# Shigangli/Ok-Topk

Hardware: NVIDIA H100
Metric: train_samples_per_sec_vgg16_oktopk_density0.001 (higher is better)
Workload: dtype fp32

## Files before the change

### oktopk_b200/csrc/bindings.cpp

```cpp
#include <pybind11/pybind11.h>
#include <pybind11/stl.h>
#include <cuda.h>
#include <cuda_runtime.h>

#include <unistd.h>

#include <algorithm>
#include <cstring>
#include <stdexcept>
#include <string>
#include <tuple>
#include <vector>

#include "oktopk.cuh"

namespace py = pybind11;
using namespace okt;

static void ck(cudaError_t e, const char* what) {
    if (e != cudaSuccess) throw std::runtime_error(std::string(what) + ": " + cudaGetErrorString(e));
}
template <class T> static T* P_(uint64_t p) { return reinterpret_cast<T*>(p); }
static cudaStream_t S_(uint64_t s) { return reinterpret_cast<cudaStream_t>(s); }

// ... 438 lines not shown
static void fused_adam(uint64_t p, uint64_t g, uint64_t m, uint64_t v, int n, double beta1, double beta2, double eps,
                       double wd, int decoupled, int zero_grad, uint64_t stream, uint64_t scal_ptr, uint64_t fault_ptr,
                       uint64_t skip_ptr) {
    if (scal_ptr == 0) throw std::runtime_error("fused_adam: scal_ptr must point at the group's device scalars");
    ck(launch_fused_adam(P_<float>(p), P_<float>(g), P_<float>(m), P_<float>(v), n, beta1, beta2, (float)eps, (float)wd,
                         decoupled, zero_grad, P_<float>(scal_ptr), P_<int>(fault_ptr), P_<int>(skip_ptr), S_(stream)),
       "fused_adam");
}
static BnDtype bn_dtype(int dtype, const char* what) {
    if (dtype < 0 || dtype > 2) throw std::runtime_error(std::string(what) + ": dtype must be 0 (fp32), 1 (bf16) or 2 (fp16)");
    return static_cast<BnDtype>(dtype);
}
static void bn_forward(uint64_t x, uint64_t y, uint64_t arg, uint64_t partial, uint64_t gamma, uint64_t beta, uint64_t cbias,
                       uint64_t save_mean, uint64_t save_invstd, uint64_t rmean, uint64_t rvar, uint64_t nbt, double momentum,
                       double eps, int relu, int M, int C, int W, int slot, int max_ctas, uint64_t stream, int dtype,
                       uint64_t res) {
    if (C % 4 != 0) throw std::runtime_error("bn_forward: channel count must be a multiple of 4");
    if (slot < 0) throw std::runtime_error("bn_forward: negative slot");
    if (res != 0 && (W != 0 || !relu)) throw std::runtime_error("bn_forward: a residual needs relu = 1 and no pool");
    ck(launch_bn_forward(P_<const void>(x), P_<void>(y), P_<unsigned char>(arg), P_<float>(partial), P_<const float>(gamma),
                         P_<const float>(beta), P_<const float>(cbias), P_<float>(save_mean), P_<float>(save_invstd),
                         P_<float>(rmean), P_<float>(rvar), P_<long long>(nbt), (float)momentum, (float)eps, relu, M, C, W, slot,
                         max_ctas, bn_dtype(dtype, "bn_forward"), S_(stream), P_<const void>(res)), "bn_forward");
}
static void bn_backward(uint64_t x, uint64_t dy, uint64_t arg, uint64_t dx, uint64_t partial, uint64_t gamma, uint64_t beta,
                        uint64_t save_mean, uint64_t save_invstd, uint64_t dgamma, uint64_t dbeta, int relu, int M, int C, int W,
                        int slot, int max_ctas, uint64_t stream, int dtype, uint64_t res, uint64_t dres) {
    if (slot < 0) throw std::runtime_error("bn_backward: negative slot");
    if ((res == 0) != (dres == 0)) throw std::runtime_error("bn_backward: res and dres go together");
    if (res != 0 && (W != 0 || !relu)) throw std::runtime_error("bn_backward: a residual needs relu = 1 and no pool");
    ck(launch_bn_backward(P_<const void>(x), P_<const void>(dy), P_<const unsigned char>(arg), P_<void>(dx), P_<float>(partial),
                          P_<const float>(gamma), P_<const float>(beta), P_<const float>(save_mean), P_<const float>(save_invstd),
                          P_<float>(dgamma), P_<float>(dbeta), relu, M, C, W, slot, max_ctas, bn_dtype(dtype, "bn_backward"),
                          S_(stream), P_<const void>(res), P_<void>(dres)), "bn_backward");
}
static void maxpool2_fwd(uint64_t x, uint64_t y, uint64_t arg, int N, int H, int W, int C, uint64_t stream) {
    if ((C % 4) || (H % 2) || (W % 2)) throw std::runtime_error("maxpool2_fwd: needs C % 4 == 0 and even H, W");
    ck(launch_maxpool2_fwd(P_<const float>(x), P_<float>(y), P_<unsigned char>(arg), N, H, W, C, S_(stream)), "maxpool2_fwd");
}
static void maxpool2_bwd(uint64_t dy, uint64_t arg, uint64_t dx, int N, int H, int W, int C, uint64_t stream) {
    ck(launch_maxpool2_bwd(P_<const float>(dy), P_<const unsigned char>(arg), P_<float>(dx), N, H, W, C, S_(stream)), "maxpool2_bwd");
}
static void momentum_correct(uint64_t g, uint64_t buf, int n, double momentum, uint64_t stream) {
    ck(launch_momentum_correct(P_<float>(g), P_<float>(buf), n, (float)momentum, S_(stream)), "momentum_correct");
}
static void clip_by_norm(uint64_t x, int n, uint64_t scratch, double max_norm, uint64_t stream) {
    ck(launch_l2norm_sq(P_<float>(x), n, P_<float>(scratch), S_(stream)), "l2norm");
    ck(launch_scale(P_<float>(x), n, P_<float>(scratch), (float)max_norm, S_(stream)), "clip scale");
}
// ... 89 lines not shown
    m.def("adam_scalars", [](uint64_t ls, uint64_t hyper, uint64_t scal, int groups, uint64_t stream) {
        ck(launch_adam_scalars(P_<const LossScaleDev>(ls), P_<const double>(hyper), P_<float>(scal), groups, S_(stream)),
           "adam_scalars");
    });
    m.def("carry_residual", [](uint64_t g, uint64_t res, int n, uint64_t skip, uint64_t stream) {
        ck(launch_carry_residual(P_<float>(g), P_<float>(res), n, P_<const int>(skip), S_(stream)), "carry_residual");
    });
    m.attr("LOSS_SCALE_BYTES") = sizeof(LossScaleDev);
    m.attr("SCALE_SYNC_BYTES") = sizeof(ScaleSync);
    m.attr("VERDICT_OFFSET") = offsetof(ScaleSync, verdict);
    m.def("maxpool2_fwd", &maxpool2_fwd);
    m.def("maxpool2_bwd", &maxpool2_bwd);
    m.def("bn_forward", &bn_forward, py::arg("x"), py::arg("y"), py::arg("arg"), py::arg("partial"), py::arg("gamma"),
          py::arg("beta"), py::arg("cbias"), py::arg("save_mean"), py::arg("save_invstd"), py::arg("rmean"), py::arg("rvar"),
          py::arg("nbt"), py::arg("momentum"), py::arg("eps"), py::arg("relu"), py::arg("M"), py::arg("C"), py::arg("W"),
          py::arg("slot"), py::arg("max_ctas"), py::arg("stream"), py::arg("dtype"), py::arg("res") = 0);
    m.def("bn_backward", &bn_backward, py::arg("x"), py::arg("dy"), py::arg("arg"), py::arg("dx"), py::arg("partial"),
          py::arg("gamma"), py::arg("beta"), py::arg("save_mean"), py::arg("save_invstd"), py::arg("dgamma"), py::arg("dbeta"),
          py::arg("relu"), py::arg("M"), py::arg("C"), py::arg("W"), py::arg("slot"), py::arg("max_ctas"), py::arg("stream"),
          py::arg("dtype"), py::arg("res") = 0, py::arg("dres") = 0);
    m.def("bn_tile_rows", &bn_tile_rows);
    m.def("clip_by_norm", &clip_by_norm);
    m.attr("MAXP") = OKT_MAXP;
    m.attr("TRACE_LEN") = kTraceLen;
    m.attr("LAND_MAX") = kLandMax;
    m.attr("SRC_SEG_MAX") = kSrcSegMax;
    m.attr("CHUNK") = kChunk;
}
```

### oktopk_b200/csrc/bnrelu.cu

```cuda
#include <cuda_bf16.h>
#include <cuda_fp16.h>

#include "common.cuh"
#include "oktopk.cuh"

namespace okt {

constexpr int kBnThreads = 256;
constexpr int kBnMaxBlocks = 512;
constexpr int kBnHold = 8;
constexpr int kBnSyncSlots = 1024;

__device__ unsigned int g_bn_sync[kBnSyncSlots][2];

struct BnGeom {
    int M, C, cv;
    int tpr, rpi;
    int rows_per_block, nblk;
    int hold;
    int W;
};

__host__ __device__ inline BnGeom bn_geom(int M, int C) {
    BnGeom g;
    g.M = M; g.C = C; g.cv = C >> 2;
    g.tpr = g.cv < kBnThreads ? g.cv : kBnThreads;
// ... 90 lines not shown
    if (ty < g.rpi) { s_red[ty * g.tpr + tx] = s; s_red[(g.rpi + ty) * g.tpr + tx] = q; }
    __syncthreads();
    if (ty == 0 && col < g.cv) {
        for (int j = 1; j < g.rpi; ++j) {
            const float4 a = s_red[j * g.tpr + tx], b = s_red[(g.rpi + j) * g.tpr + tx];
            s.x += a.x; s.y += a.y; s.z += a.z; s.w += a.w;
            q.x += b.x; q.y += b.y; q.z += b.z; q.w += b.w;
        }
        float4* p4 = reinterpret_cast<float4*>(partial + (size_t)tile * 2 * g.C);
        p4[col] = s;
        p4[g.cv + col] = q;
    }
    __syncthreads();
}

__device__ __forceinline__ bool bn_arrive(unsigned int* sync, unsigned int& gen) {
    __shared__ unsigned int s_gen;
    __shared__ int s_last;
    __syncthreads();
    if (threadIdx.x == 0) {
        s_gen = ld_acquire_gpu_u32(sync + 1);
        const unsigned int old = atom_add_acq_rel_gpu_u32(sync, 1u);
        s_last = old == gridDim.x - 1u;
        if (s_last) st_relaxed_gpu_u32(sync, 0u);
    }
    __syncthreads();
    gen = s_gen;
    return s_last != 0;
}

__device__ __forceinline__ void bn_release(unsigned int* sync, bool last, unsigned int gen) {
    __syncthreads();
    if (threadIdx.x == 0) {
        if (last) {
            st_release_gpu_u32(sync + 1, gen + 1u);
        } else {
            while (ld_acquire_gpu_u32(sync + 1) == gen) { }
        }
    }
    __syncthreads();
}

template <typename T>
struct BnFwdArgs {
    const T* x;
    T* y;
    unsigned char* arg;
    float* partial;
    const float* gamma; const float* beta; const float* cbias;
    float* save_mean; float* save_invstd; float* rmean; float* rvar; long long* nbt;
    float momentum, eps;
    int relu;
    unsigned int* sync;
    BnGeom g;
    const T* res;
};

template <bool kPool, bool kRes, typename T>
__global__ void __launch_bounds__(kBnThreads) bn_fwd_kernel(const BnFwdArgs<T> p) {
    static_assert(!(kPool && kRes), "no pool follows a residual add");
    using A = BnAct<T>;
    using V = typename A::V;
    extern __shared__ float4 s_dyn[];
    __shared__ float4 s_red[2 * kBnThreads];
    const BnGeom& g = p.g;
    const int tx = threadIdx.x % g.tpr, ty = threadIdx.x / g.tpr;
    const V* x4 = reinterpret_cast<const V*>(p.x);
    auto ldx = [&](size_t o) { return A::wide(__ldg(x4 + o)); };
    const size_t st1 = (size_t)g.rpi * g.cv;
    V h[kBnHold];

    for (int t = blockIdx.x; t < g.nblk; t += gridDim.x) {
        const bool held = g.hold && t == (int)blockIdx.x;
        const int row0 = t * g.rows_per_block, row1 = min(g.M, row0 + g.rows_per_block);
        for (int c0 = 0; c0 < g.cv; c0 += g.tpr) {
            const int col = c0 + tx;
            float4 s = make_float4(0.f, 0.f, 0.f, 0.f), q = s;
            if (ty < g.rpi && col < g.cv) {
                auto acc = [&](const float4& v) {
                    s.x += v.x; s.y += v.y; s.z += v.z; s.w += v.w;
// ... 9 lines not shown
                        if (r + k * g.rpi < row1) acc(A::wide(h[k]));
                } else {
                    for (; r + 3 * g.rpi < row1; r += 4 * g.rpi) {
                        const size_t o = (size_t)r * g.cv + col;
                        const float4 v0 = ldx(o), v1 = ldx(o + st1), v2 = ldx(o + 2 * st1), v3 = ldx(o + 3 * st1);
                        acc(v0); acc(v1); acc(v2); acc(v3);
                    }
                    for (; r < row1; r += g.rpi) acc(ldx((size_t)r * g.cv + col));
                }
            }
            bn_tile_partial(s, q, tx, ty, col, g, s_red, p.partial, t);
        }
    }

    float* s_ab = reinterpret_cast<float*>(s_dyn);
    unsigned int gen;
    const bool last = bn_arrive(p.sync, gen);
    if (last) {
        float* s_tot = s_ab;
        bn_combine_partials(p.partial, g.nblk, g.C, s_tot, s_red);
        for (int c = threadIdx.x; c < g.C; c += kBnThreads) {
            const double s = (double)s_tot[c], q = (double)s_tot[g.C + c];
            const double mean = s / (double)g.M;
            double var = q / (double)g.M - mean * mean;
            if (var < 0.0) var = 0.0;
            const float invstd = (float)(1.0 / sqrt(var + (double)p.eps));
            p.save_mean[c] = (float)mean;
            p.save_invstd[c] = invstd;
            if (p.rmean != nullptr) {
                const float mb = (float)mean + (p.cbias != nullptr ? __ldg(p.cbias + c) : 0.f);
                const double unb = g.M > 1 ? var * (double)g.M / (double)(g.M - 1) : var;
                p.rmean[c] = fmaf(p.momentum, mb, __fmul_rn(1.f - p.momentum, p.rmean[c]));
                p.rvar[c] = fmaf(p.momentum, (float)unb, __fmul_rn(1.f - p.momentum, p.rvar[c]));
            }
        }
        if (threadIdx.x == 0 && p.nbt != nullptr) *p.nbt += 1;
    }
    bn_release(p.sync, last, gen);
    for (int c = threadIdx.x; c < g.C; c += kBnThreads) {
        const float a = __fmul_rn(__ldg(p.gamma + c), __ldcg(p.save_invstd + c));
        s_ab[c] = a;
        s_ab[g.C + c] = __fsub_rn(__ldg(p.beta + c), __fmul_rn(__ldcg(p.save_mean + c), a));
    }
    __syncthreads();

    const float4* ab4 = s_dyn;
    auto yval = [&](const float4& xin, int col) {
        float4 v = f4_fma(xin, ab4[col], ab4[g.cv + col]);
        if (p.relu) { v.x = fmaxf(v.x, 0.f); v.y = fmaxf(v.y, 0.f); v.z = fmaxf(v.z, 0.f); v.w = fmaxf(v.w, 0.f); }
        return v;
    };
    const V* r4 = reinterpret_cast<const V*>(p.res);
    auto ldr = [&](size_t o) { return A::wide(__ldg(r4 + o)); };
    auto yres = [&](const float4& xin, const float4& rin, int col) {
        float4 v = f4_fma(xin, ab4[col], ab4[g.cv + col]);
        v.x += rin.x; v.y += rin.y; v.z += rin.z; v.w += rin.w;
        v.x = fmaxf(v.x, 0.f); v.y = fmaxf(v.y, 0.f); v.z = fmaxf(v.z, 0.f); v.w = fmaxf(v.w, 0.f);
// ... 77 lines not shown
struct BnBwdArgs {
    const T* x;
    const T* dy;
    const unsigned char* arg;
    T* dx;
    float* partial;
    const float* gamma; const float* beta; const float* save_mean; const float* save_invstd;
    float* dgamma; float* dbeta;
    int relu;
    unsigned int* sync;
    BnGeom g;
    const T* res;
    T* dres;
};

template <bool kPool, bool kRes, typename T>
__global__ void __launch_bounds__(kBnThreads) bn_bwd_kernel(const BnBwdArgs<T> p) {
    static_assert(!(kPool && kRes), "no pool follows a residual add");
    using A = BnAct<T>;
    using V = typename A::V;
    extern __shared__ float4 s_dyn[];
    __shared__ float4 s_red[2 * kBnThreads];
    const BnGeom& g = p.g;
    const int tx = threadIdx.x % g.tpr, ty = threadIdx.x / g.tpr;
    const V* x4 = reinterpret_cast<const V*>(p.x);
    const V* d4 = reinterpret_cast<const V*>(p.dy);
    const uchar4* a4 = reinterpret_cast<const uchar4*>(p.arg);
    auto ldx = [&](size_t o) { return A::wide(__ldg(x4 + o)); };
    const size_t st1 = (size_t)g.rpi * g.cv;
    auto grad = [&](int row0, int r, int col) -> float4 {
        if (!kPool) return A::wide(__ldg(d4 + (size_t)r * g.cv + col));
        const int lr = r - row0, hl = lr / g.W, w = lr - hl * g.W;
        const size_t o = (size_t)(row0 / 4 + (hl >> 1) * (g.W >> 1) + (w >> 1)) * g.cv + col;
        const int k = (hl & 1) * 2 + (w & 1);
        const float4 d = A::wide(__ldg(d4 + o));
        const uchar4 a = __ldg(a4 + o);
        return make_float4(a.x == k ? d.x : 0.f, a.y == k ? d.y : 0.f, a.z == k ? d.z : 0.f, a.w == k ? d.w : 0.f);
    };
// ... 85 lines not shown
                            const size_t o = (size_t)r * g.cv + col;
                            const float4 v = ldx(o);
                            float4 e = grad(row0, r, col);
                            gate(k, v, ldr(o), o, e);
                            acc(v, e);
                        } else {
                            acc(ldx((size_t)r * g.cv + col), grad(row0, r, col));
                        }
                    }
                }
            }
            bn_tile_partial(sb, sg, tx, ty, col, g, s_red, p.partial, t);
        }
    }

    unsigned int gen;
    const bool last = bn_arrive(p.sync, gen);
    if (last) {
        float* s_tot = reinterpret_cast<float*>(s_dyn);
        bn_combine_partials(p.partial, g.nblk, g.C, s_tot, s_red);
        for (int c = threadIdx.x; c < g.C; c += kBnThreads) { p.dbeta[c] = s_tot[c]; p.dgamma[c] = s_tot[g.C + c]; }
    }
    bn_release(p.sync, last, gen);

    for (int t = blockIdx.x; t < g.nblk; t += gridDim.x) {
        const bool held = g.hold && t == (int)blockIdx.x;
        const int row0 = t * g.rows_per_block, row1 = min(g.M, row0 + g.rows_per_block);
        for (int c0 = 0; c0 < g.cv; c0 += g.tpr) {
            const int col = c0 + tx;
            if (ty >= g.rpi || col >= g.cv) continue;
            const Col k = column(col);
            const float4 db = __ldcg(reinterpret_cast<const float4*>(p.dbeta) + col);
            const float4 dg = __ldcg(reinterpret_cast<const float4*>(p.dgamma) + col);
            const double M = (double)g.M;
            const float4 mb = make_float4((float)(db.x / M), (float)(db.y / M), (float)(db.z / M), (float)(db.w / M));
            const float4 mg = make_float4((float)(dg.x / M), (float)(dg.y / M), (float)(dg.z / M), (float)(dg.w / M));
            V* o4 = reinterpret_cast<V*>(p.dx);
            auto out = [&](size_t off, const float4& v, float4 d) {
                const float4 xh = xhat(k, v);
                if constexpr (!kRes) mask(k, v, d);
                o4[off] = A::narrow(make_float4(k.a.x * (d.x - mb.x - xh.x * mg.x), k.a.y * (d.y - mb.y - xh.y * mg.y),
                                                k.a.z * (d.z - mb.z - xh.z * mg.z), k.a.w * (d.w - mb.w - xh.w * mg.w)));
            };
            int r = row0 + ty;
            if (held) {
#pragma unroll
                for (int j = 0; j < kBnHold; ++j)
                    if (r + j * g.rpi < row1) out((size_t)(r + j * g.rpi) * g.cv + col, A::wide(hx[j]), hd[j]);
// ... 18 lines not shown

static unsigned int* bn_sync_slot(int slot) {
    static unsigned int* base[64] = {nullptr};
    int dev = 0;
    cudaGetDevice(&dev);
    if (dev < 0 || dev >= 64) return nullptr;
    if (base[dev] == nullptr) {
        void* a = nullptr;
        if (cudaGetSymbolAddress(&a, g_bn_sync) != cudaSuccess) return nullptr;
        base[dev] = static_cast<unsigned int*>(a);
    }
    return base[dev] + 2 * (size_t)(slot % kBnSyncSlots);
}

template <typename Args>
static cudaError_t bn_launch(void (*kernel)(const Args), Args p, size_t smem, int max_ctas, cudaStream_t stream) {
    int dev = 0, sms = 0, per = 0;
    cudaGetDevice(&dev);
    cudaError_t e = cudaDeviceGetAttribute(&sms, cudaDevAttrMultiProcessorCount, dev);
    if (e == cudaSuccess && smem > 32 * 1024)
        e = cudaFuncSetAttribute(kernel, cudaFuncAttributeMaxDynamicSharedMemorySize, (int)smem);
    if (e == cudaSuccess) e = cudaOccupancyMaxActiveBlocksPerMultiprocessor(&per, kernel, kBnThreads, smem);
    if (e != cudaSuccess) return e;
    if (per < 1) return cudaErrorInvalidConfiguration;
    int grid = p.g.nblk < per * sms ? p.g.nblk : per * sms;
    if (max_ctas > 0 && grid > max_ctas) grid = max_ctas;
    void* args[] = {(void*)&p};
    e = cudaLaunchCooperativeKernel((void*)kernel, dim3(grid), dim3(kBnThreads), args, smem, stream);
    (void)cudaGetLastError();
    return e;
}

static cudaError_t bn_prepare(BnGeom& g, unsigned int*& sync, int M, int C, int W, int slot) {
    g = bn_geom(M, C);
    g.W = W;
    if (W > 0 && (W % 2 != 0 || g.rows_per_block % (2 * W) != 0 || M % (2 * W) != 0)) return cudaErrorInvalidValue;
    sync = bn_sync_slot(slot);
    return sync == nullptr ? cudaErrorInvalidDevice : cudaSuccess;
}

template <typename T>
static cudaError_t bn_forward_t(const void* x, void* y, unsigned char* arg, float* partial, const float* gamma,
                                const float* beta, const float* cbias, float* save_mean, float* save_invstd, float* rmean,
                                float* rvar, long long* nbt, float momentum, float eps, int relu, int M, int C, int W, int slot,
                                int max_ctas, cudaStream_t stream, const void* res) {
    if (res != nullptr && (W > 0 || !relu)) return cudaErrorInvalidValue;
    BnFwdArgs<T> p{static_cast<const T*>(x), static_cast<T*>(y), arg, partial, gamma, beta, cbias, save_mean, save_invstd,
                   rmean, rvar, nbt, momentum, eps, relu, nullptr, {}, static_cast<const T*>(res)};
    cudaError_t e = bn_prepare(p.g, p.sync, M, C, W, slot);
    if (e != cudaSuccess) return e;
    size_t smem = sizeof(float) * 2 * C;
    if (W > 0 && p.g.hold) smem += sizeof(float4) * p.g.rows_per_block * p.g.cv;
    if (W > 0) return bn_launch(bn_fwd_kernel<true, false, T>, p, smem, max_ctas, stream);
    return res != nullptr ? bn_launch(bn_fwd_kernel<false, true, T>, p, smem, max_ctas, stream)
                          : bn_launch(bn_fwd_kernel<false, false, T>, p, smem, max_ctas, stream);
}

template <typename T>
static cudaError_t bn_backward_t(const void* x, const void* dy, const unsigned char* arg, void* dx, float* partial,
                                 const float* gamma, const float* beta, const float* save_mean, const float* save_invstd,
                                 float* dgamma, float* dbeta, int relu, int M, int C, int W, int slot, int max_ctas,
                                 cudaStream_t stream, const void* res, void* dres) {
    if ((res == nullptr) != (dres == nullptr) || (res != nullptr && (W > 0 || !relu))) return cudaErrorInvalidValue;
    BnBwdArgs<T> p{static_cast<const T*>(x), static_cast<const T*>(dy), arg, static_cast<T*>(dx), partial, gamma, beta,
                   save_mean, save_invstd, dgamma, dbeta, relu, nullptr, {}, static_cast<const T*>(res),
                   static_cast<T*>(dres)};
    cudaError_t e = bn_prepare(p.g, p.sync, M, C, W, slot);
    if (e != cudaSuccess) return e;
    const size_t smem = sizeof(float) * 2 * C;
    if (W > 0) return bn_launch(bn_bwd_kernel<true, false, T>, p, smem, max_ctas, stream);
    return res != nullptr ? bn_launch(bn_bwd_kernel<false, true, T>, p, smem, max_ctas, stream)
                          : bn_launch(bn_bwd_kernel<false, false, T>, p, smem, max_ctas, stream);
}

cudaError_t launch_bn_forward(const void* x, void* y, unsigned char* arg, float* partial, const float* gamma, const float* beta,
                              const float* cbias, float* save_mean, float* save_invstd, float* rmean, float* rvar, long long* nbt,
                              float momentum, float eps, int relu, int M, int C, int W, int slot, int max_ctas, BnDtype dtype,
                              cudaStream_t stream, const void* res) {
    switch (dtype) {
        case BnDtype::kF32:
            return bn_forward_t<float>(x, y, arg, partial, gamma, beta, cbias, save_mean, save_invstd, rmean, rvar, nbt,
                                       momentum, eps, relu, M, C, W, slot, max_ctas, stream, res);
        case BnDtype::kBF16:
            return bn_forward_t<__nv_bfloat16>(x, y, arg, partial, gamma, beta, cbias, save_mean, save_invstd, rmean, rvar,
                                               nbt, momentum, eps, relu, M, C, W, slot, max_ctas, stream, res);
        case BnDtype::kF16:
            return bn_forward_t<__half>(x, y, arg, partial, gamma, beta, cbias, save_mean, save_invstd, rmean, rvar, nbt,
                                        momentum, eps, relu, M, C, W, slot, max_ctas, stream, res);
    }
    return cudaErrorInvalidValue;
}

cudaError_t launch_bn_backward(const void* x, const void* dy, const unsigned char* arg, void* dx, float* partial,
                               const float* gamma, const float* beta, const float* save_mean, const float* save_invstd,
                               float* dgamma, float* dbeta, int relu, int M, int C, int W, int slot, int max_ctas, BnDtype dtype,
                               cudaStream_t stream, const void* res, void* dres) {
    switch (dtype) {
        case BnDtype::kF32:
            return bn_backward_t<float>(x, dy, arg, dx, partial, gamma, beta, save_mean, save_invstd, dgamma, dbeta, relu,
                                        M, C, W, slot, max_ctas, stream, res, dres);
        case BnDtype::kBF16:
            return bn_backward_t<__nv_bfloat16>(x, dy, arg, dx, partial, gamma, beta, save_mean, save_invstd, dgamma, dbeta,
                                                relu, M, C, W, slot, max_ctas, stream, res, dres);
        case BnDtype::kF16:
            return bn_backward_t<__half>(x, dy, arg, dx, partial, gamma, beta, save_mean, save_invstd, dgamma, dbeta, relu,
                                         M, C, W, slot, max_ctas, stream, res, dres);
    }
    return cudaErrorInvalidValue;
}

}

namespace okt {

constexpr int kPoolThreads = 256;

__global__ void __launch_bounds__(kPoolThreads) maxpool2_fwd_kernel(const float* __restrict__ x, float* __restrict__ y,
                                                                     unsigned char* __restrict__ arg, int N, int H, int W,
                                                                     int C) {
    const int cv = C >> 2, Ho = H >> 1, Wo = W >> 1;
    const long long total = (long long)N * Ho * Wo * cv;
// ... 70 lines not shown
```

### oktopk_b200/csrc/common.cuh

```cuda
#pragma once
#include <cuda_runtime.h>
#include <stdint.h>

#ifndef OKT_MAXP
#define OKT_MAXP 16
#endif

namespace okt {

__device__ __forceinline__ unsigned long long globaltimer_ns() {
    unsigned long long t;
    asm volatile("mov.u64 %0, %%globaltimer;" : "=l"(t));
    return t;
}

__device__ __forceinline__ void st_release_sys_u64(uint64_t* p, uint64_t v) {
    asm volatile("st.release.sys.global.u64 [%0], %1;" ::"l"(p), "l"(v) : "memory");
}
__device__ __forceinline__ uint64_t ld_acquire_sys_u64(const uint64_t* p) {
    uint64_t v;
    asm volatile("ld.acquire.sys.global.u64 %0, [%1];" : "=l"(v) : "l"(p) : "memory");
    return v;
}
__device__ __forceinline__ uint64_t ld_relaxed_sys_u64(const uint64_t* p) {
// ... 8 lines not shown
    asm volatile("st.relaxed.sys.global.u64 [%0], %1;" ::"l"(p), "l"(v) : "memory");
}
__device__ __forceinline__ uint32_t ld_relaxed_sys_u32(const uint32_t* p) {
    uint32_t v;
    asm volatile("ld.relaxed.sys.global.u32 %0, [%1];" : "=r"(v) : "l"(p) : "memory");
    return v;
}
__device__ __forceinline__ unsigned long long ld_acquire_gpu_u64(const unsigned long long* p) {
    unsigned long long v;
    asm volatile("ld.acquire.gpu.global.u64 %0, [%1];" : "=l"(v) : "l"(p) : "memory");
    return v;
}
__device__ __forceinline__ uint32_t ld_acquire_gpu_u32(const uint32_t* p) {
    uint32_t v;
    asm volatile("ld.acquire.gpu.global.u32 %0, [%1];" : "=r"(v) : "l"(p) : "memory");
    return v;
}
__device__ __forceinline__ void st_release_gpu_u32(uint32_t* p, uint32_t v) {
    asm volatile("st.release.gpu.global.u32 [%0], %1;" ::"l"(p), "r"(v) : "memory");
}
__device__ __forceinline__ void st_relaxed_gpu_u32(uint32_t* p, uint32_t v) {
    asm volatile("st.relaxed.gpu.global.u32 [%0], %1;" ::"l"(p), "r"(v) : "memory");
}
__device__ __forceinline__ uint32_t atom_add_acq_rel_gpu_u32(uint32_t* p, uint32_t v) {
    uint32_t old;
    asm volatile("atom.acq_rel.gpu.global.add.u32 %0, [%1], %2;" : "=r"(old) : "l"(p), "r"(v) : "memory");
    return old;
}
__device__ __forceinline__ void fence_acq_rel_sys() { asm volatile("fence.acq_rel.sys;" ::: "memory"); }
__device__ __forceinline__ void fence_acq_rel_gpu() { asm volatile("fence.acq_rel.gpu;" ::: "memory"); }
// ... 189 lines not shown
```

### oktopk_b200/csrc/oktopk.cuh

```cuda
#pragma once
#include <cuda_runtime.h>
#include <stdint.h>
#include <stddef.h>

#ifndef OKT_MAXP
#define OKT_MAXP 16
#endif

namespace okt {

constexpr int kThreads = 512;
constexpr int kWarps = kThreads / 32;
constexpr int kChunk = 1024;
constexpr int kHistBins = 2048;
constexpr int kMaxWarpsTotal = 16384;
constexpr int kGuardMax = 64;
constexpr int kGuardFineMax = 15;
constexpr int kCtasPerSm = 1;
constexpr int kPackTile = 2;
constexpr int kPackStages = 4;
constexpr int kPackSmemBytes = kPackStages * 2 * kPackTile * kThreads * 16;
constexpr int kScanStages = 2 * kPackStages;
constexpr int kStrideGridMax = 132 * 8;

// ... 262 lines not shown
cudaError_t launch_carry_residual(float* g, float* res, int n, const int* skip, cudaStream_t stream);
constexpr int kLandMax = 96;
struct LandParams {
    const float* src[kLandMax];
    long long dst_off[kLandMax];
    int numel[kLandMax];
    int blk_begin[kLandMax + 1];
    int count;
};
cudaError_t launch_land(const LandParams& lp, float* bucket, cudaStream_t stream);
enum class BnDtype : int { kF32 = 0, kBF16 = 1, kF16 = 2 };
int bn_tile_rows(int M, int C);
cudaError_t launch_bn_forward(const void* x, void* y, unsigned char* arg, float* partial, const float* gamma, const float* beta,
                              const float* cbias, float* save_mean, float* save_invstd, float* rmean, float* rvar, long long* nbt,
                              float momentum, float eps, int relu, int M, int C, int W, int slot, int max_ctas, BnDtype dtype,
                              cudaStream_t stream, const void* res = nullptr);
cudaError_t launch_bn_backward(const void* x, const void* dy, const unsigned char* arg, void* dx, float* partial,
                               const float* gamma, const float* beta, const float* save_mean, const float* save_invstd,
                               float* dgamma, float* dbeta, int relu, int M, int C, int W, int slot, int max_ctas, BnDtype dtype,
                               cudaStream_t stream, const void* res = nullptr, void* dres = nullptr);
cudaError_t launch_maxpool2_fwd(const float* x, float* y, unsigned char* arg, int N, int H, int W, int C, cudaStream_t stream);
cudaError_t launch_maxpool2_bwd(const float* dy, const unsigned char* arg, float* dx, int N, int H, int W, int C,
                                cudaStream_t stream);
cudaError_t launch_momentum_correct(float* g, float* buf, int n, float momentum, cudaStream_t stream);
cudaError_t launch_l2norm_sq(const float* x, int n, float* out, cudaStream_t stream);
cudaError_t launch_scale(float* x, int n, const float* norm_sq, float max_norm, cudaStream_t stream);

}
```

### oktopk_b200/ops/fused_bn.py

```python
from __future__ import annotations

import itertools
from typing import Optional

import torch
import torch.nn.functional as F

from . import ext

MAX_CTAS = 0

_SLOTS = itertools.count()

_DTYPE_FLAG = {torch.float32: 0, torch.bfloat16: 1, torch.float16: 2}


def _sync_slot(bn: torch.nn.BatchNorm2d) -> int:
    s = bn.__dict__.get("_okt_bn_slot")
    if s is None:
        s = bn.__dict__["_okt_bn_slot"] = next(_SLOTS)
    return s


def _dtype_ok(x: torch.Tensor, fp16: bool = False) -> bool:
    if not torch.is_autocast_enabled():
# ... 40 lines not shown
        dtype = _DTYPE_FLAG[x.dtype]
        if pool:
            y = torch.empty((N, Ch, H // 2, W // 2), dtype=x.dtype, device=x.device, memory_format=torch.channels_last)
            arg = torch.empty(y.numel(), dtype=torch.uint8, device=x.device)
        else:
            y = torch.empty_like(x)
            arg = None
        rows = C.bn_tile_rows(M, Ch)
        partial = torch.empty((M + rows - 1) // rows * 2 * Ch, dtype=torch.float32, device=x.device)
        stats = torch.empty(2 * Ch, dtype=torch.float32, device=x.device)
        s = torch.cuda.current_stream().cuda_stream
        C.bn_forward(x.data_ptr(), y.data_ptr(), 0 if arg is None else arg.data_ptr(), partial.data_ptr(), gamma.data_ptr(),
                     beta.data_ptr(), 0 if cbias is None else cbias.data_ptr(), stats.data_ptr(), stats.data_ptr() + 4 * Ch,
                     0 if rmean is None else rmean.data_ptr(), 0 if rvar is None else rvar.data_ptr(),
                     0 if nbt is None else nbt.data_ptr(), float(momentum), float(eps), int(relu), M, Ch,
                     W if pool else 0, slot, MAX_CTAS, s, dtype, 0 if res is None else res.data_ptr())
        ctx.save_for_backward(x, gamma, beta, stats, arg, res)
        ctx.relu, ctx.pool, ctx.slot, ctx.dtype = bool(relu), bool(pool), slot, dtype
        return y

    @staticmethod
    def backward(ctx, dy):
        C = ext.require()
        x, gamma, beta, stats, arg, res = ctx.saved_tensors
        N, Ch, H, W = x.shape
        M = N * H * W
        assert dy.dtype == x.dtype, (dy.dtype, x.dtype)
        if not dy.is_contiguous(memory_format=torch.channels_last):
            dy = dy.contiguous(memory_format=torch.channels_last)
        dx = torch.empty_like(x)
        rows = C.bn_tile_rows(M, Ch)
        partial = torch.empty((M + rows - 1) // rows * 2 * Ch, dtype=torch.float32, device=x.device)
        dgb = torch.empty(2 * Ch, dtype=torch.float32, device=x.device)
        dres = None if res is None else torch.empty_like(x)
        s = torch.cuda.current_stream().cuda_stream
        C.bn_backward(x.data_ptr(), dy.data_ptr(), 0 if arg is None else arg.data_ptr(), dx.data_ptr(), partial.data_ptr(),
                      gamma.data_ptr(), beta.data_ptr(), stats.data_ptr(), stats.data_ptr() + 4 * Ch, dgb.data_ptr(),
                      dgb.data_ptr() + 4 * Ch, int(ctx.relu), M, Ch, W if ctx.pool else 0, ctx.slot, MAX_CTAS, s,
                      ctx.dtype, 0 if res is None else res.data_ptr(), 0 if dres is None else dres.data_ptr())
        return dx, dgb[:Ch], dgb[Ch:], None, None, None, None, None, None, None, None, None, dres


def _check_residual(residual: Optional[torch.Tensor], relu: bool, pool: Optional[torch.nn.MaxPool2d]) -> None:
    if residual is not None and (not relu or pool is not None):
        raise ValueError("a residual is added before the ReLU: it needs relu=True and pool=None")


def bias_bn_relu(x: torch.Tensor, bn: torch.nn.BatchNorm2d, conv_bias: Optional[torch.Tensor] = None,
                 relu: bool = True, pool: Optional[torch.nn.MaxPool2d] = None, fp16: bool = False,
                 residual: Optional[torch.Tensor] = None) -> torch.Tensor:
    _check_residual(residual, relu, pool)
    if (_fast_path_ok(x, bn, fp16) and (conv_bias is None or conv_bias.dtype == torch.float32)
            and (residual is None or _residual_ok(x, residual))):
        if residual is not None and not residual.is_contiguous(memory_format=torch.channels_last):
# ... 96 lines not shown
```

Before: 13160.

## Let every CTA combine BN partials redundantly instead of last-block broadcast

Adds a variant of the fused BN forward and backward kernels in which every CTA waits at a grid barrier and then reduces all per-tile partials itself. The last CTA alone writes saved stats, running stats and dgamma/dbeta, while every CTA uses its own shared-memory copy. The old scheme had a serial combine by one CTA and a second global read of the stats after release. The variant is chosen when the tile count is at most 128, and it trades redundant reduction reads of the partials for a shorter critical path.

```diff
diff --git a/oktopk_b200/csrc/bindings.cpp b/oktopk_b200/csrc/bindings.cpp
--- a/oktopk_b200/csrc/bindings.cpp
+++ b/oktopk_b200/csrc/bindings.cpp
@@ -476,25 +476,25 @@
 static void bn_forward(uint64_t x, uint64_t y, uint64_t arg, uint64_t partial, uint64_t gamma, uint64_t beta, uint64_t cbias,
                        uint64_t save_mean, uint64_t save_invstd, uint64_t rmean, uint64_t rvar, uint64_t nbt, double momentum,
                        double eps, int relu, int M, int C, int W, int slot, int max_ctas, uint64_t stream, int dtype,
-                       uint64_t res) {
+                       uint64_t res, int all_tiles) {
     if (C % 4 != 0) throw std::runtime_error("bn_forward: channel count must be a multiple of 4");
     if (slot < 0) throw std::runtime_error("bn_forward: negative slot");
     if (res != 0 && (W != 0 || !relu)) throw std::runtime_error("bn_forward: a residual needs relu = 1 and no pool");
     ck(launch_bn_forward(P_<const void>(x), P_<void>(y), P_<unsigned char>(arg), P_<float>(partial), P_<const float>(gamma),
                          P_<const float>(beta), P_<const float>(cbias), P_<float>(save_mean), P_<float>(save_invstd),
                          P_<float>(rmean), P_<float>(rvar), P_<long long>(nbt), (float)momentum, (float)eps, relu, M, C, W, slot,
-                         max_ctas, bn_dtype(dtype, "bn_forward"), S_(stream), P_<const void>(res)), "bn_forward");
+                         max_ctas, bn_dtype(dtype, "bn_forward"), S_(stream), P_<const void>(res), all_tiles), "bn_forward");
 }
 static void bn_backward(uint64_t x, uint64_t dy, uint64_t arg, uint64_t dx, uint64_t partial, uint64_t gamma, uint64_t beta,
                         uint64_t save_mean, uint64_t save_invstd, uint64_t dgamma, uint64_t dbeta, int relu, int M, int C, int W,
-                        int slot, int max_ctas, uint64_t stream, int dtype, uint64_t res, uint64_t dres) {
+                        int slot, int max_ctas, uint64_t stream, int dtype, uint64_t res, uint64_t dres, int all_tiles) {
     if (slot < 0) throw std::runtime_error("bn_backward: negative slot");
     if ((res == 0) != (dres == 0)) throw std::runtime_error("bn_backward: res and dres go together");
     if (res != 0 && (W != 0 || !relu)) throw std::runtime_error("bn_backward: a residual needs relu = 1 and no pool");
     ck(launch_bn_backward(P_<const void>(x), P_<const void>(dy), P_<const unsigned char>(arg), P_<void>(dx), P_<float>(partial),
                           P_<const float>(gamma), P_<const float>(beta), P_<const float>(save_mean), P_<const float>(save_invstd),
                           P_<float>(dgamma), P_<float>(dbeta), relu, M, C, W, slot, max_ctas, bn_dtype(dtype, "bn_backward"),
-                          S_(stream), P_<const void>(res), P_<void>(dres)), "bn_backward");
+                          S_(stream), P_<const void>(res), P_<void>(dres), all_tiles), "bn_backward");
 }
 static void maxpool2_fwd(uint64_t x, uint64_t y, uint64_t arg, int N, int H, int W, int C, uint64_t stream) {
     if ((C % 4) || (H % 2) || (W % 2)) throw std::runtime_error("maxpool2_fwd: needs C % 4 == 0 and even H, W");
@@ -614,11 +614,12 @@
     m.def("bn_forward", &bn_forward, py::arg("x"), py::arg("y"), py::arg("arg"), py::arg("partial"), py::arg("gamma"),
           py::arg("beta"), py::arg("cbias"), py::arg("save_mean"), py::arg("save_invstd"), py::arg("rmean"), py::arg("rvar"),
           py::arg("nbt"), py::arg("momentum"), py::arg("eps"), py::arg("relu"), py::arg("M"), py::arg("C"), py::arg("W"),
-          py::arg("slot"), py::arg("max_ctas"), py::arg("stream"), py::arg("dtype"), py::arg("res") = 0);
+          py::arg("slot"), py::arg("max_ctas"), py::arg("stream"), py::arg("dtype"), py::arg("res") = 0,
+          py::arg("all_tiles") = -1);
     m.def("bn_backward", &bn_backward, py::arg("x"), py::arg("dy"), py::arg("arg"), py::arg("dx"), py::arg("partial"),
           py::arg("gamma"), py::arg("beta"), py::arg("save_mean"), py::arg("save_invstd"), py::arg("dgamma"), py::arg("dbeta"),
           py::arg("relu"), py::arg("M"), py::arg("C"), py::arg("W"), py::arg("slot"), py::arg("max_ctas"), py::arg("stream"),
-          py::arg("dtype"), py::arg("res") = 0, py::arg("dres") = 0);
+          py::arg("dtype"), py::arg("res") = 0, py::arg("dres") = 0, py::arg("all_tiles") = -1);
     m.def("bn_tile_rows", &bn_tile_rows);
     m.def("clip_by_norm", &clip_by_norm);
     m.attr("MAXP") = OKT_MAXP;
diff --git a/oktopk_b200/csrc/bnrelu.cu b/oktopk_b200/csrc/bnrelu.cu
--- a/oktopk_b200/csrc/bnrelu.cu
+++ b/oktopk_b200/csrc/bnrelu.cu
@@ -10,6 +10,8 @@
 constexpr int kBnMaxBlocks = 512;
 constexpr int kBnHold = 8;
 constexpr int kBnSyncSlots = 1024;
+
+constexpr int kBnAllCombineTiles = 128;
 
 __device__ unsigned int g_bn_sync[kBnSyncSlots][2];
 
@@ -130,19 +132,55 @@
     __syncthreads();
 }
 
-__device__ __forceinline__ bool bn_arrive(unsigned int* sync, unsigned int& gen) {
-    __shared__ unsigned int s_gen;
+__device__ __forceinline__ unsigned int bn_gen(const unsigned int* sync) {
+    return threadIdx.x == 0 ? ld_relaxed_gpu_u32(sync + 1) : 0u;
+}
+
+__device__ __forceinline__ bool bn_arrive(unsigned int* sync) {
     __shared__ int s_last;
     __syncthreads();
     if (threadIdx.x == 0) {
-        s_gen = ld_acquire_gpu_u32(sync + 1);
         const unsigned int old = atom_add_acq_rel_gpu_u32(sync, 1u);
         s_last = old == gridDim.x - 1u;
         if (s_last) st_relaxed_gpu_u32(sync, 0u);
     }
     __syncthreads();
-    gen = s_gen;
     return s_last != 0;
+}
+
+__device__ __forceinline__ bool bn_arrive_all(unsigned int* sync, unsigned int gen) {
+    __shared__ int s_last;
+    __syncthreads();
+    if (threadIdx.x == 0) {
+        const unsigned int old = atom_add_acq_rel_gpu_u32(sync, 1u);
+        const bool last = old == gridDim.x - 1u;
+        if (last) {
+            st_relaxed_gpu_u32(sync, 0u);
+            st_release_gpu_u32(sync + 1, gen + 1u);
+        } else {
+            while (ld_acquire_gpu_u32(sync + 1) == gen) { }
+        }
+        s_last = last;
+    }
+    __syncthreads();
+    return s_last != 0;
+}
+
+struct BnStat { float mean, invstd; double var; };
+__device__ __forceinline__ BnStat bn_stat(float s_, float q_, int M, float eps) {
+    const double s = (double)s_, q = (double)q_;
+    const double mean = s / (double)M;
+    BnStat r;
+    r.var = q / (double)M - mean * mean;
+    if (r.var < 0.0) r.var = 0.0;
+    r.mean = (float)mean;
+    r.invstd = (float)(1.0 / sqrt(r.var + (double)eps));
+    return r;
+}
+
+__device__ __forceinline__ void bn_ab(float gamma, float beta, float mean, float invstd, float& a, float& b) {
+    a = __fmul_rn(gamma, invstd);
+    b = __fsub_rn(beta, __fmul_rn(mean, a));
 }
 
 __device__ __forceinline__ void bn_release(unsigned int* sync, bool last, unsigned int gen) {
@@ -172,7 +210,20 @@
     const T* res;
 };
 
-template <bool kPool, bool kRes, typename T>
+template <typename T>
+__device__ __forceinline__ void bn_save_stat(const BnFwdArgs<T>& p, int c, const BnStat& st) {
+    p.save_mean[c] = st.mean;
+    p.save_invstd[c] = st.invstd;
+    if (p.rmean != nullptr) {
+        const int M = p.g.M;
+        const float mb = st.mean + (p.cbias != nullptr ? __ldg(p.cbias + c) : 0.f);
+        const double unb = M > 1 ? st.var * (double)M / (double)(M - 1) : st.var;
+        p.rmean[c] = fmaf(p.momentum, mb, __fmul_rn(1.f - p.momentum, p.rmean[c]));
+        p.rvar[c] = fmaf(p.momentum, (float)unb, __fmul_rn(1.f - p.momentum, p.rvar[c]));
+    }
+}
+
+template <bool kAll, bool kPool, bool kRes, typename T>
 __global__ void __launch_bounds__(kBnThreads) bn_fwd_kernel(const BnFwdArgs<T> p) {
     static_assert(!(kPool && kRes), "no pool follows a residual add");
     using A = BnAct<T>;
@@ -180,6 +231,7 @@
     extern __shared__ float4 s_dyn[];
     __shared__ float4 s_red[2 * kBnThreads];
     const BnGeom& g = p.g;
+    const unsigned int gen = bn_gen(p.sync);
     const int tx = threadIdx.x % g.tpr, ty = threadIdx.x / g.tpr;
     const V* x4 = reinterpret_cast<const V*>(p.x);
     auto ldx = [&](size_t o) { return A::wide(__ldg(x4 + o)); };
@@ -219,33 +271,28 @@
     }
 
     float* s_ab = reinterpret_cast<float*>(s_dyn);
-    unsigned int gen;
-    const bool last = bn_arrive(p.sync, gen);
-    if (last) {
+    if constexpr (!kAll) {
+        const bool last = bn_arrive(p.sync);
+        if (last) {
+            float* s_tot = s_ab;
+            bn_combine_partials(p.partial, g.nblk, g.C, s_tot, s_red);
+            for (int c = threadIdx.x; c < g.C; c += kBnThreads) bn_save_stat(p, c, bn_stat(s_tot[c], s_tot[g.C + c], g.M, p.eps));
+            if (threadIdx.x == 0 && p.nbt != nullptr) *p.nbt += 1;
+        }
+        bn_release(p.sync, last, gen);
+        for (int c = threadIdx.x; c < g.C; c += kBnThreads)
+            bn_ab(__ldg(p.gamma + c), __ldg(p.beta + c), __ldcg(p.save_mean + c), __ldcg(p.save_invstd + c), s_ab[c],
+                  s_ab[g.C + c]);
+    } else {
         float* s_tot = s_ab;
+        const bool writer = bn_arrive_all(p.sync, gen);
         bn_combine_partials(p.partial, g.nblk, g.C, s_tot, s_red);
         for (int c = threadIdx.x; c < g.C; c += kBnThreads) {
-            const double s = (double)s_tot[c], q = (double)s_tot[g.C + c];
-            const double mean = s / (double)g.M;
-            double var = q / (double)g.M - mean * mean;
-            if (var < 0.0) var = 0.0;
-            const float invstd = (float)(1.0 / sqrt(var + (double)p.eps));
-            p.save_mean[c] = (float)mean;
-            p.save_invstd[c] = invstd;
-            if (p.rmean != nullptr) {
-                const float mb = (float)mean + (p.cbias != nullptr ? __ldg(p.cbias + c) : 0.f);
-                const double unb = g.M > 1 ? var * (double)g.M / (double)(g.M - 1) : var;
-                p.rmean[c] = fmaf(p.momentum, mb, __fmul_rn(1.f - p.momentum, p.rmean[c]));
-                p.rvar[c] = fmaf(p.momentum, (float)unb, __fmul_rn(1.f - p.momentum, p.rvar[c]));
-            }
-        }
-        if (threadIdx.x == 0 && p.nbt != nullptr) *p.nbt += 1;
-    }
-    bn_release(p.sync, last, gen);
-    for (int c = threadIdx.x; c < g.C; c += kBnThreads) {
-        const float a = __fmul_rn(__ldg(p.gamma + c), __ldcg(p.save_invstd + c));
-        s_ab[c] = a;
-        s_ab[g.C + c] = __fsub_rn(__ldg(p.beta + c), __fmul_rn(__ldcg(p.save_mean + c), a));
+            const BnStat st = bn_stat(s_tot[c], s_tot[g.C + c], g.M, p.eps);
+            if (writer) bn_save_stat(p, c, st);
+            bn_ab(__ldg(p.gamma + c), __ldg(p.beta + c), st.mean, st.invstd, s_ab[c], s_ab[g.C + c]);
+        }
+        if (writer && threadIdx.x == 0 && p.nbt != nullptr) *p.nbt += 1;
     }
     __syncthreads();
 
@@ -353,7 +400,7 @@
     T* dres;
 };
 
-template <bool kPool, bool kRes, typename T>
+template <bool kAll, bool kPool, bool kRes, typename T>
 __global__ void __launch_bounds__(kBnThreads) bn_bwd_kernel(const BnBwdArgs<T> p) {
     static_assert(!(kPool && kRes), "no pool follows a residual add");
     using A = BnAct<T>;
@@ -361,6 +408,8 @@
     extern __shared__ float4 s_dyn[];
     __shared__ float4 s_red[2 * kBnThreads];
     const BnGeom& g = p.g;
+    const unsigned int gen = bn_gen(p.sync);
+    float* s_tot = reinterpret_cast<float*>(s_dyn);
     const int tx = threadIdx.x % g.tpr, ty = threadIdx.x / g.tpr;
     const V* x4 = reinterpret_cast<const V*>(p.x);
     const V* d4 = reinterpret_cast<const V*>(p.dy);
@@ -476,14 +525,28 @@
         }
     }
 
-    unsigned int gen;
-    const bool last = bn_arrive(p.sync, gen);
-    if (last) {
-        float* s_tot = reinterpret_cast<float*>(s_dyn);
+    if constexpr (!kAll) {
+        const bool last = bn_arrive(p.sync);
+        if (last) {
+            bn_combine_partials(p.partial, g.nblk, g.C, s_tot, s_red);
+            for (int c = threadIdx.x; c < g.C; c += kBnThreads) { p.dbeta[c] = s_tot[c]; p.dgamma[c] = s_tot[g.C + c]; }
+        }
+        bn_release(p.sync, last, gen);
+    } else {
+        const bool writer = bn_arrive_all(p.sync, gen);
         bn_combine_partials(p.partial, g.nblk, g.C, s_tot, s_red);
-        for (int c = threadIdx.x; c < g.C; c += kBnThreads) { p.dbeta[c] = s_tot[c]; p.dgamma[c] = s_tot[g.C + c]; }
-    }
-    bn_release(p.sync, last, gen);
+        if (writer)
+            for (int c = threadIdx.x; c < g.C; c += kBnThreads) { p.dbeta[c] = s_tot[c]; p.dgamma[c] = s_tot[g.C + c]; }
+    }
+    auto dbeta_dgamma = [&](int col, float4& db, float4& dg) {
+        if constexpr (!kAll) {
+            db = __ldcg(reinterpret_cast<const float4*>(p.dbeta) + col);
+            dg = __ldcg(reinterpret_cast<const float4*>(p.dgamma) + col);
+        } else {
+            db = reinterpret_cast<const float4*>(s_tot)[col];
+            dg = reinterpret_cast<const float4*>(s_tot)[g.cv + col];
+        }
+    };
 
     for (int t = blockIdx.x; t < g.nblk; t += gridDim.x) {
         const bool held = g.hold && t == (int)blockIdx.x;
@@ -492,8 +555,8 @@
             const int col = c0 + tx;
             if (ty >= g.rpi || col >= g.cv) continue;
             const Col k = column(col);
-            const float4 db = __ldcg(reinterpret_cast<const float4*>(p.dbeta) + col);
-            const float4 dg = __ldcg(reinterpret_cast<const float4*>(p.dgamma) + col);
+            float4 db, dg;
+            dbeta_dgamma(col, db, dg);
             const double M = (double)g.M;
             const float4 mb = make_float4((float)(db.x / M), (float)(db.y / M), (float)(db.z / M), (float)(db.w / M));
             const float4 mg = make_float4((float)(dg.x / M), (float)(dg.y / M), (float)(dg.z / M), (float)(dg.w / M));
@@ -542,7 +605,9 @@
 }
 
 template <typename Args>
-static cudaError_t bn_launch(void (*kernel)(const Args), Args p, size_t smem, int max_ctas, cudaStream_t stream) {
+static cudaError_t bn_launch(void (*k_one)(const Args), void (*k_all)(const Args), Args p, size_t smem, int max_ctas,
+                             int all_tiles, cudaStream_t stream) {
+    void (*kernel)(const Args) = p.g.nblk <= (all_tiles >= 0 ? all_tiles : kBnAllCombineTiles) ? k_all : k_one;
     int dev = 0, sms = 0, per = 0;
     cudaGetDevice(&dev);
     cudaError_t e = cudaDeviceGetAttribute(&sms, cudaDevAttrMultiProcessorCount, dev);
@@ -567,11 +632,23 @@
     return sync == nullptr ? cudaErrorInvalidDevice : cudaSuccess;
 }
 
+template <bool kPool, bool kRes, typename T>
+static cudaError_t bn_fwd_launch(const BnFwdArgs<T>& p, size_t smem, int max_ctas, int all_tiles, cudaStream_t stream) {
+    return bn_launch(bn_fwd_kernel<false, kPool, kRes, T>, bn_fwd_kernel<true, kPool, kRes, T>, p, smem, max_ctas, all_tiles,
+                     stream);
+}
+
+template <bool kPool, bool kRes, typename T>
+static cudaError_t bn_bwd_launch(const BnBwdArgs<T>& p, size_t smem, int max_ctas, int all_tiles, cudaStream_t stream) {
+    return bn_launch(bn_bwd_kernel<false, kPool, kRes, T>, bn_bwd_kernel<true, kPool, kRes, T>, p, smem, max_ctas, all_tiles,
+                     stream);
+}
+
 template <typename T>
 static cudaError_t bn_forward_t(const void* x, void* y, unsigned char* arg, float* partial, const float* gamma,
                                 const float* beta, const float* cbias, float* save_mean, float* save_invstd, float* rmean,
                                 float* rvar, long long* nbt, float momentum, float eps, int relu, int M, int C, int W, int slot,
-                                int max_ctas, cudaStream_t stream, const void* res) {
+                                int max_ctas, cudaStream_t stream, const void* res, int all_tiles) {
     if (res != nullptr && (W > 0 || !relu)) return cudaErrorInvalidValue;
     BnFwdArgs<T> p{static_cast<const T*>(x), static_cast<T*>(y), arg, partial, gamma, beta, cbias, save_mean, save_invstd,
                    rmean, rvar, nbt, momentum, eps, relu, nullptr, {}, static_cast<const T*>(res)};
@@ -579,16 +656,16 @@
     if (e != cudaSuccess) return e;
     size_t smem = sizeof(float) * 2 * C;
     if (W > 0 && p.g.hold) smem += sizeof(float4) * p.g.rows_per_block * p.g.cv;
-    if (W > 0) return bn_launch(bn_fwd_kernel<true, false, T>, p, smem, max_ctas, stream);
-    return res != nullptr ? bn_launch(bn_fwd_kernel<false, true, T>, p, smem, max_ctas, stream)
-                          : bn_launch(bn_fwd_kernel<false, false, T>, p, smem, max_ctas, stream);
+    if (W > 0) return bn_fwd_launch<true, false>(p, smem, max_ctas, all_tiles, stream);
+    return res != nullptr ? bn_fwd_launch<false, true>(p, smem, max_ctas, all_tiles, stream)
+                          : bn_fwd_launch<false, false>(p, smem, max_ctas, all_tiles, stream);
 }
 
 template <typename T>
 static cudaError_t bn_backward_t(const void* x, const void* dy, const unsigned char* arg, void* dx, float* partial,
                                  const float* gamma, const float* beta, const float* save_mean, const float* save_invstd,
                                  float* dgamma, float* dbeta, int relu, int M, int C, int W, int slot, int max_ctas,
-                                 cudaStream_t stream, const void* res, void* dres) {
+                                 cudaStream_t stream, const void* res, void* dres, int all_tiles) {
     if ((res == nullptr) != (dres == nullptr) || (res != nullptr && (W > 0 || !relu))) return cudaErrorInvalidValue;
     BnBwdArgs<T> p{static_cast<const T*>(x), static_cast<const T*>(dy), arg, static_cast<T*>(dx), partial, gamma, beta,
                    save_mean, save_invstd, dgamma, dbeta, relu, nullptr, {}, static_cast<const T*>(res),
@@ -596,25 +673,25 @@
     cudaError_t e = bn_prepare(p.g, p.sync, M, C, W, slot);
     if (e != cudaSuccess) return e;
     const size_t smem = sizeof(float) * 2 * C;
-    if (W > 0) return bn_launch(bn_bwd_kernel<true, false, T>, p, smem, max_ctas, stream);
-    return res != nullptr ? bn_launch(bn_bwd_kernel<false, true, T>, p, smem, max_ctas, stream)
-                          : bn_launch(bn_bwd_kernel<false, false, T>, p, smem, max_ctas, stream);
+    if (W > 0) return bn_bwd_launch<true, false>(p, smem, max_ctas, all_tiles, stream);
+    return res != nullptr ? bn_bwd_launch<false, true>(p, smem, max_ctas, all_tiles, stream)
+                          : bn_bwd_launch<false, false>(p, smem, max_ctas, all_tiles, stream);
 }
 
 cudaError_t launch_bn_forward(const void* x, void* y, unsigned char* arg, float* partial, const float* gamma, const float* beta,
                               const float* cbias, float* save_mean, float* save_invstd, float* rmean, float* rvar, long long* nbt,
                               float momentum, float eps, int relu, int M, int C, int W, int slot, int max_ctas, BnDtype dtype,
-                              cudaStream_t stream, const void* res) {
+                              cudaStream_t stream, const void* res, int all_tiles) {
     switch (dtype) {
         case BnDtype::kF32:
             return bn_forward_t<float>(x, y, arg, partial, gamma, beta, cbias, save_mean, save_invstd, rmean, rvar, nbt,
-                                       momentum, eps, relu, M, C, W, slot, max_ctas, stream, res);
+                                       momentum, eps, relu, M, C, W, slot, max_ctas, stream, res, all_tiles);
         case BnDtype::kBF16:
             return bn_forward_t<__nv_bfloat16>(x, y, arg, partial, gamma, beta, cbias, save_mean, save_invstd, rmean, rvar,
-                                               nbt, momentum, eps, relu, M, C, W, slot, max_ctas, stream, res);
+                                               nbt, momentum, eps, relu, M, C, W, slot, max_ctas, stream, res, all_tiles);
         case BnDtype::kF16:
             return bn_forward_t<__half>(x, y, arg, partial, gamma, beta, cbias, save_mean, save_invstd, rmean, rvar, nbt,
-                                        momentum, eps, relu, M, C, W, slot, max_ctas, stream, res);
+                                        momentum, eps, relu, M, C, W, slot, max_ctas, stream, res, all_tiles);
     }
     return cudaErrorInvalidValue;
 }
@@ -622,17 +699,17 @@
 cudaError_t launch_bn_backward(const void* x, const void* dy, const unsigned char* arg, void* dx, float* partial,
                                const float* gamma, const float* beta, const float* save_mean, const float* save_invstd,
                                float* dgamma, float* dbeta, int relu, int M, int C, int W, int slot, int max_ctas, BnDtype dtype,
-                               cudaStream_t stream, const void* res, void* dres) {
+                               cudaStream_t stream, const void* res, void* dres, int all_tiles) {
     switch (dtype) {
         case BnDtype::kF32:
             return bn_backward_t<float>(x, dy, arg, dx, partial, gamma, beta, save_mean, save_invstd, dgamma, dbeta, relu,
-                                        M, C, W, slot, max_ctas, stream, res, dres);
+                                        M, C, W, slot, max_ctas, stream, res, dres, all_tiles);
         case BnDtype::kBF16:
             return bn_backward_t<__nv_bfloat16>(x, dy, arg, dx, partial, gamma, beta, save_mean, save_invstd, dgamma, dbeta,
-                                                relu, M, C, W, slot, max_ctas, stream, res, dres);
+                                                relu, M, C, W, slot, max_ctas, stream, res, dres, all_tiles);
         case BnDtype::kF16:
             return bn_backward_t<__half>(x, dy, arg, dx, partial, gamma, beta, save_mean, save_invstd, dgamma, dbeta, relu,
-                                         M, C, W, slot, max_ctas, stream, res, dres);
+                                         M, C, W, slot, max_ctas, stream, res, dres, all_tiles);
     }
     return cudaErrorInvalidValue;
 }
diff --git a/oktopk_b200/csrc/common.cuh b/oktopk_b200/csrc/common.cuh
--- a/oktopk_b200/csrc/common.cuh
+++ b/oktopk_b200/csrc/common.cuh
@@ -46,6 +46,11 @@
 __device__ __forceinline__ uint32_t ld_acquire_gpu_u32(const uint32_t* p) {
     uint32_t v;
     asm volatile("ld.acquire.gpu.global.u32 %0, [%1];" : "=r"(v) : "l"(p) : "memory");
+    return v;
+}
+__device__ __forceinline__ uint32_t ld_relaxed_gpu_u32(const uint32_t* p) {
+    uint32_t v;
+    asm volatile("ld.relaxed.gpu.global.u32 %0, [%1];" : "=r"(v) : "l"(p) : "memory");
     return v;
 }
 __device__ __forceinline__ void st_release_gpu_u32(uint32_t* p, uint32_t v) {
diff --git a/oktopk_b200/csrc/oktopk.cuh b/oktopk_b200/csrc/oktopk.cuh
--- a/oktopk_b200/csrc/oktopk.cuh
+++ b/oktopk_b200/csrc/oktopk.cuh
@@ -300,11 +300,11 @@
 cudaError_t launch_bn_forward(const void* x, void* y, unsigned char* arg, float* partial, const float* gamma, const float* beta,
                               const float* cbias, float* save_mean, float* save_invstd, float* rmean, float* rvar, long long* nbt,
                               float momentum, float eps, int relu, int M, int C, int W, int slot, int max_ctas, BnDtype dtype,
-                              cudaStream_t stream, const void* res = nullptr);
+                              cudaStream_t stream, const void* res = nullptr, int all_tiles = -1);
 cudaError_t launch_bn_backward(const void* x, const void* dy, const unsigned char* arg, void* dx, float* partial,
                                const float* gamma, const float* beta, const float* save_mean, const float* save_invstd,
                                float* dgamma, float* dbeta, int relu, int M, int C, int W, int slot, int max_ctas, BnDtype dtype,
-                               cudaStream_t stream, const void* res = nullptr, void* dres = nullptr);
+                               cudaStream_t stream, const void* res = nullptr, void* dres = nullptr, int all_tiles = -1);
 cudaError_t launch_maxpool2_fwd(const float* x, float* y, unsigned char* arg, int N, int H, int W, int C, cudaStream_t stream);
 cudaError_t launch_maxpool2_bwd(const float* dy, const unsigned char* arg, float* dx, int N, int H, int W, int C,
                                 cudaStream_t stream);
diff --git a/oktopk_b200/ops/fused_bn.py b/oktopk_b200/ops/fused_bn.py
--- a/oktopk_b200/ops/fused_bn.py
+++ b/oktopk_b200/ops/fused_bn.py
@@ -9,6 +9,8 @@
 from . import ext
 
 MAX_CTAS = 0
+
+ALL_COMBINE_TILES = -1
 
 _SLOTS = itertools.count()
 
@@ -79,7 +81,8 @@
                      beta.data_ptr(), 0 if cbias is None else cbias.data_ptr(), stats.data_ptr(), stats.data_ptr() + 4 * Ch,
                      0 if rmean is None else rmean.data_ptr(), 0 if rvar is None else rvar.data_ptr(),
                      0 if nbt is None else nbt.data_ptr(), float(momentum), float(eps), int(relu), M, Ch,
-                     W if pool else 0, slot, MAX_CTAS, s, dtype, 0 if res is None else res.data_ptr())
+                     W if pool else 0, slot, MAX_CTAS, s, dtype, 0 if res is None else res.data_ptr(),
+                     all_tiles=ALL_COMBINE_TILES)
         ctx.save_for_backward(x, gamma, beta, stats, arg, res)
         ctx.relu, ctx.pool, ctx.slot, ctx.dtype = bool(relu), bool(pool), slot, dtype
         return y
@@ -102,7 +105,8 @@
         C.bn_backward(x.data_ptr(), dy.data_ptr(), 0 if arg is None else arg.data_ptr(), dx.data_ptr(), partial.data_ptr(),
                       gamma.data_ptr(), beta.data_ptr(), stats.data_ptr(), stats.data_ptr() + 4 * Ch, dgb.data_ptr(),
                       dgb.data_ptr() + 4 * Ch, int(ctx.relu), M, Ch, W if ctx.pool else 0, ctx.slot, MAX_CTAS, s,
-                      ctx.dtype, 0 if res is None else res.data_ptr(), 0 if dres is None else dres.data_ptr())
+                      ctx.dtype, 0 if res is None else res.data_ptr(), 0 if dres is None else dres.data_ptr(),
+                      all_tiles=ALL_COMBINE_TILES)
         return dx, dgb[:Ch], dgb[Ch:], None, None, None, None, None, None, None, None, None, dres
 
 
```

Measured after the change: 13460 (median of 6 runs). About the same (+2.2%).
